# PrimeIntellect-ai/prime

Hardware: AMD Instinct MI355X
Metric: tokens_per_sec (higher is better)
Workload: dtype bf16; 1 GPU; model=intellect_10b, global_batch=8, seq_len=2048, parallelism=diloco1_h100_int8ring

## Files before the change

prime_amd/ops/_lib.py:

```python
from __future__ import annotations

import ctypes
from typing import Optional

import torch

from .build import LIB_PATH, build, needs_build

_LIB: Optional[ctypes.CDLL] = None
_TRIED = False

_SIGS = {
    "prime_rmsnorm_fwd": [ctypes.c_void_p] * 5 + [ctypes.c_int64] * 2 + [ctypes.c_double],
    "prime_rmsnorm_bwd": [ctypes.c_void_p] * 7 + [ctypes.c_int64] * 3 + [ctypes.c_double],
    "prime_add_rmsnorm_fwd": [ctypes.c_void_p] * 7 + [ctypes.c_int64] * 2 + [ctypes.c_double],
    "prime_add_rmsnorm_bwd": [ctypes.c_void_p] * 8 + [ctypes.c_int64] * 3 + [ctypes.c_double],
    "prime_rope": [ctypes.c_void_p] * 5 + [ctypes.c_int64] * 4 + [ctypes.c_int, ctypes.c_int64, ctypes.c_void_p],
    "prime_rope_strided": [ctypes.c_void_p] * 5 + [ctypes.c_int64] * 7,
    "prime_qkv_grad_pack": [ctypes.c_void_p] * 8 + [ctypes.c_int64] * 6,
    "prime_swiglu_bwd_t": [ctypes.c_void_p] * 5 + [ctypes.c_int64] * 2,
    "prime_swiglu_fwd": [ctypes.c_void_p] * 3 + [ctypes.c_int64] * 2,
    "prime_swiglu_bwd": [ctypes.c_void_p] * 4 + [ctypes.c_int64] * 2,
    "prime_adamw": [ctypes.c_void_p] * 7 + [ctypes.c_int64] + [ctypes.c_double] * 5 + [ctypes.c_int64],
    "prime_grad_sqnorm": [ctypes.c_void_p] * 3 + [ctypes.c_int64] * 2,
    "prime_grad_sqnorm_partials": [],
    "prime_pseudograd": [ctypes.c_void_p] * 4 + [ctypes.c_int64],
    "prime_quant_int8": [ctypes.c_void_p] * 4 + [ctypes.c_int64],
    "prime_dequant_int8": [ctypes.c_void_p] * 4 + [ctypes.c_int64] * 2,
    "prime_nesterov_outer": [ctypes.c_void_p] * 6 + [ctypes.c_int64] + [ctypes.c_double] * 2,
    "prime_cross_entropy": [ctypes.c_void_p] * 5 + [ctypes.c_int64] * 2 + [ctypes.c_double] + [ctypes.c_int64] * 2,
    "prime_flash_fwd": [ctypes.c_void_p] * 6 + [ctypes.c_int64] * 5 + [ctypes.c_double] + [ctypes.c_int64] * 7 + [ctypes.c_void_p],
    "prime_attn_delta": [ctypes.c_void_p] * 4 + [ctypes.c_int64] * 2,
    "prime_flash_bwd_dq": [ctypes.c_void_p] * 9 + [ctypes.c_int64] * 5 + [ctypes.c_double] + [ctypes.c_int64] * 10 + [ctypes.c_void_p],
    "prime_flash_bwd_dkv": [ctypes.c_void_p] * 13 + [ctypes.c_int64] * 6 + [ctypes.c_double] + [ctypes.c_int64] * 10 + [ctypes.c_void_p],
    "prime_mfma_probe": [ctypes.c_void_p] * 4,
    "prime_mfma_probe32": [ctypes.c_void_p] * 4,
    "prime_transpose_bshd": [ctypes.c_void_p] * 3 + [ctypes.c_int64] * 7,
    "prime_attn_decode": [ctypes.c_void_p] * 5 + [ctypes.c_int64] * 6 + [ctypes.c_double, ctypes.c_void_p],
    "prime_attn_decode_ragged": [ctypes.c_void_p] * 7 + [ctypes.c_int64] * 6 + [ctypes.c_double],
    "prime_decode_ragged_chunk": [],
    "prime_decode_qkv_append": [ctypes.c_void_p] * 8 + [ctypes.c_int64] * 6,
    "prime_gemm_nt": [ctypes.c_void_p] * 4 + [ctypes.c_int64] * 4,
    "prime_gemm_nt8": [ctypes.c_void_p] * 4 + [ctypes.c_int64] * 4,
    "prime_quant_fp8": [ctypes.c_void_p] * 6 + [ctypes.c_int64] * 2,
    "prime_rowwise_quant_fp8": [ctypes.c_void_p] * 4 + [ctypes.c_int64] * 3,
    "prime_transpose_fp8": [ctypes.c_void_p] * 3 + [ctypes.c_int64] * 7 + [ctypes.c_void_p] * 3 + [ctypes.c_int64],
}


def _load() -> ctypes.CDLL:
    import os

    override = os.environ.get("PRIME_AMD_LIB_PATH")
    path = override or str(LIB_PATH)
    if override is None and needs_build():
        build(verbose=True)
    lib = ctypes.CDLL(path)
    for name, argtypes in _SIGS.items():
        try:
            fn = getattr(lib, name)
        except AttributeError:
            continue
        fn.argtypes = argtypes
        fn.restype = ctypes.c_int
    return lib


def lib() -> ctypes.CDLL:
    global _LIB, _TRIED
    if _LIB is None:
        if _TRIED:
            raise RuntimeError("prime_amd HIP kernel library failed to load earlier")
        _TRIED = True
        try:
            _LIB = _load()
        except Exception as e:
            raise RuntimeError(
                "prime_amd requires its HIP kernel library on GPU machines; "
                f"build failed or .so missing at {LIB_PATH}: {e}"
            ) from e
    return _LIB


def have_lib() -> bool:
    try:
        lib()
        return True
# ... 19 lines not shown
```

prime_amd/ops/csrc/attention.hip:

```cpp
#include "common.h"
#include <stdlib.h>

typedef __attribute__((ext_vector_type(8))) short short8;
typedef __attribute__((ext_vector_type(4))) float f32x4;
typedef __attribute__((address_space(3))) char lds_char;
typedef __attribute__((address_space(3))) void lds_void;
typedef __attribute__((address_space(1))) const void g_void;

__device__ __forceinline__ short8 ld8(const bf16* p) {
  return *reinterpret_cast<const short8*>(p);
}

__device__ __forceinline__ f32x4 mfma16(short8 a, short8 b, f32x4 c) {
  return __builtin_amdgcn_mfma_f32_16x16x32_bf16(a, b, c, 0, 0, 0);
}

__device__ __forceinline__ float grp16_max(float x) {
#pragma unroll
  for (int off = 1; off < 16; off <<= 1) x = fmaxf(x, __shfl_xor(x, off, 64));
  return x;
}
__device__ __forceinline__ float grp16_sum(float x) {
#pragma unroll
  for (int off = 1; off < 16; off <<= 1) x += __shfl_xor(x, off, 64);
// ... 370 lines not shown
        psum += pv;
      }
    psum += __shfl_xor(psum, 32, 64);
    l_run = l_run * alpha + psum;

    short8 pa[2 * 2];
#pragma unroll
    for (int t = 0; t < 2; ++t) {
#pragma unroll
      for (int kst = 0; kst < 2; ++kst) {
        const int g0 = 4 * (2 * kst), g1 = 4 * (2 * kst + 1);
        unsigned x0 = cvt_pk_bf16(st[t][g0 + 0], st[t][g0 + 1]);
        unsigned x1 = cvt_pk_bf16(st[t][g0 + 2], st[t][g0 + 3]);
        unsigned y0 = cvt_pk_bf16(st[t][g1 + 0], st[t][g1 + 1]);
        unsigned y1 = cvt_pk_bf16(st[t][g1 + 2], st[t][g1 + 3]);
        permlane32_swap(x0, y0);
        permlane32_swap(x1, y1);
        short8 frag;
        reinterpret_cast<unsigned*>(&frag)[0] = x0;
        reinterpret_cast<unsigned*>(&frag)[1] = x1;
        reinterpret_cast<unsigned*>(&frag)[2] = y0;
        reinterpret_cast<unsigned*>(&frag)[3] = y1;
        pa[t * 2 + kst] = frag;
      }
    }
    if (FLAGS & 1) __builtin_amdgcn_s_setprio(1);
#pragma unroll
    for (int dt = 0; dt < DT32; ++dt)
#pragma unroll
      for (int ks = 0; ks < 4; ++ks)
        o_acc[dt] = mfma32(pa[ks],
                           ld8_swz<64>(vt_lds[idx], dt * 32 + lo, ks * 32 + hi * 16),
                           o_acc[dt]);
    if (FLAGS & 1) __builtin_amdgcn_s_setprio(0);
  }
  if (hi == 0) bcast[lo] = (l_run > 0.f) ? 1.f / l_run : 0.f;
  wave_lds_fence();
#pragma unroll
  for (int r = 0; r < 16; ++r) {
    const int qr = (r & 3) + 8 * (r >> 2) + 4 * hi;
    const float inv = bcast[qr];
    bf16* orow = O + (((int64_t)(b * S + q0w + qr)) * H + h) * D;
#pragma unroll
    for (int dt = 0; dt < DT32; ++dt)
      orow[dt * 32 + lo] = f2bf(o_acc[dt][r] * inv);
  }
  if (hi == 0)
    lse[((int64_t)(b * S + q0w + lo)) * H + h] = m_run + __logf(fmaxf(l_run, 1e-30f));
}

__global__ void attn_delta_kernel(const bf16* __restrict__ dO,
                                  const bf16* __restrict__ O,
                                  float* __restrict__ delta, int64_t rows,
                                  int D) {
  const int64_t row0 = (int64_t)blockIdx.x * (blockDim.x >> 6) + (threadIdx.x >> 6);
  const int lane = threadIdx.x & 63;
  for (int64_t r = row0; r < rows; r += (int64_t)gridDim.x * (blockDim.x >> 6)) {
    float acc = 0.f;
    for (int i = lane * 2; i < D; i += 128) {
      acc += bf2f(dO[r * D + i]) * bf2f(O[r * D + i]);
      acc += bf2f(dO[r * D + i + 1]) * bf2f(O[r * D + i + 1]);
    }
    acc = wave_reduce_sum(acc);
    if (lane == 0) delta[r] = acc;
  }
}

template <int D, int FLAGS, bool DOC = false>
__global__ __launch_bounds__(512, 2) void flash_bwd_dq_v5_kernel(
    const bf16* __restrict__ Q, const bf16* __restrict__ K,
    const bf16* __restrict__ V, const bf16* __restrict__ Kt,
    const bf16* __restrict__ dO, const float* __restrict__ lse,
    const float* __restrict__ delta, bf16* __restrict__ dQ, int B, int H,
    int Hkv, int S, float scale, int causal,
    int64_t sqb, int64_t sqs, int64_t sqh,
    int64_t skb, int64_t sks, int64_t skh,
    int64_t svb, int64_t svs, int64_t svh,
    const int* __restrict__ doc) {
  constexpr int DSL = D / 16;
  constexpr int DT32 = D / 32;
  const int n_qt = S / 256;
  const int nwg = gridDim.x;
  int vb = blockIdx.x;
  if ((nwg & 7) == 0) vb = (blockIdx.x & 7) * (nwg >> 3) + (blockIdx.x >> 3);
  const int bh = vb / n_qt;
  const int qt = n_qt - 1 - (vb - bh * n_qt);
  const int b = bh / H, h = bh - b * H;
  const int hkv = h / (H / Hkv);
  const int wid = threadIdx.x >> 6;
  const int lane = threadIdx.x & 63;
  const int lo = lane & 31, hi = lane >> 5;
  const int q0w = qt * 256 + wid * 32;

  const bf16* Qb = Q + b * sqb + h * sqh;
  const bf16* Kb = K + b * skb + hkv * skh;
  const bf16* Vb = V + b * svb + hkv * svh;
  const bf16* Ktb = Kt + ((int64_t)(b * Hkv + hkv) * D) * S;
  const bf16* dOb = dO + ((int64_t)b * S * H + h) * D;
  const float* lse_b = lse + (int64_t)b * S * H + h;
  const float* dl_b = delta + (int64_t)b * S * H + h;

  __shared__ bf16 k_lds[2][64 * D];
  __shared__ bf16 v_lds[2][64 * D];
  __shared__ bf16 kt_lds[2][D * 64];

  short8 qf[DSL], dof[DSL];
#pragma unroll
  for (int ds = 0; ds < DSL; ++ds) {
    const bf16* src = Qb + (int64_t)(q0w + lo) * sqs + ds * 16 + hi * 8;
    short8 raw = ld8(src);
    short8 sc;
#pragma unroll
    for (int j = 0; j < 8; ++j) {
      bf16 v = reinterpret_cast<const bf16*>(&raw)[j];
      reinterpret_cast<bf16*>(&sc)[j] = f2bf(bf2f(v) * scale);
    }
    qf[ds] = sc;
// ... 308 lines not shown
        const int g0 = 4 * (2 * kst), g1 = 4 * (2 * kst + 1);
        unsigned x0 = cvt_pk_bf16(st[g0 + 0], st[g0 + 1]);
        unsigned x1 = cvt_pk_bf16(st[g0 + 2], st[g0 + 3]);
        unsigned y0 = cvt_pk_bf16(st[g1 + 0], st[g1 + 1]);
        unsigned y1 = cvt_pk_bf16(st[g1 + 2], st[g1 + 3]);
        permlane32_swap(x0, y0);
        permlane32_swap(x1, y1);
        short8 f;
        reinterpret_cast<unsigned*>(&f)[0] = x0;
        reinterpret_cast<unsigned*>(&f)[1] = x1;
        reinterpret_cast<unsigned*>(&f)[2] = y0;
        reinterpret_cast<unsigned*>(&f)[3] = y1;
        pa[kst] = f;
        x0 = cvt_pk_bf16(dpt[g0 + 0], dpt[g0 + 1]);
        x1 = cvt_pk_bf16(dpt[g0 + 2], dpt[g0 + 3]);
        y0 = cvt_pk_bf16(dpt[g1 + 0], dpt[g1 + 1]);
        y1 = cvt_pk_bf16(dpt[g1 + 2], dpt[g1 + 3]);
        permlane32_swap(x0, y0);
        permlane32_swap(x1, y1);
        reinterpret_cast<unsigned*>(&f)[0] = x0;
        reinterpret_cast<unsigned*>(&f)[1] = x1;
        reinterpret_cast<unsigned*>(&f)[2] = y0;
        reinterpret_cast<unsigned*>(&f)[3] = y1;
        da[kst] = f;
      }
      if (FLAGS & 1) __builtin_amdgcn_s_setprio(1);
#pragma unroll
      for (int dt = 0; dt < DT32; ++dt)
#pragma unroll
        for (int kst = 0; kst < 2; ++kst) {
          const int colb = qs * 64 + kst * 32 + hi * 16;
          dv_acc[dt] = mfma32(pa[kst],
                              ld8_swz<64>(dot_lds[cur], dt * 32 + lo, colb),
                              dv_acc[dt]);
          dk_acc[dt] = mfma32(da[kst],
                              ld8_swz<64>(qt_lds[cur], dt * 32 + lo, colb),
                              dk_acc[dt]);
        }
      if (FLAGS & 1) __builtin_amdgcn_s_setprio(0);
    }
  }
#pragma unroll
  for (int r = 0; r < 16; ++r) {
    const int kg = k0w + (r & 3) + 8 * (r >> 2) + 4 * hi;
    const int64_t base = ((((int64_t)split * B + b) * Hkv + hkv) * S + kg) * D;
#pragma unroll
    for (int dt = 0; dt < DT32; ++dt) {
      wsK[base + dt * 32 + lo] = dk_acc[dt][r];
      wsV[base + dt * 32 + lo] = dv_acc[dt][r];
    }
  }
}

template <int D, int NW = 4, int DBUF = 1, bool DOC = false>
__global__ __launch_bounds__(512) void flash_bwd_dkv_kernel(
    const bf16* __restrict__ Q, const bf16* __restrict__ Qt,
    const bf16* __restrict__ K, const bf16* __restrict__ V,
    const bf16* __restrict__ dO, const bf16* __restrict__ dOt,
    const float* __restrict__ lse, const float* __restrict__ delta,
    float* __restrict__ wsK, float* __restrict__ wsV, int B, int H, int Hkv,
    int S, float scale, int causal, int splits,
    int64_t sqb, int64_t sqs, int64_t sqh,
    int64_t skb, int64_t sks, int64_t skh,
    int64_t svb, int64_t svs, int64_t svh,
    const int* __restrict__ doc_end) {
  constexpr int DS = D / 32;
  constexpr int DT = D / 16;
  const int n_kt = S / (NW * 16);
  const int per_split = (B * Hkv) * n_kt;
  const int split = blockIdx.x / per_split;
  const int rem = blockIdx.x - split * per_split;
  const int bh = rem / n_kt;
  const int kt = rem - bh * n_kt;
  const int b = bh / Hkv, hkv = bh - b * Hkv;
  const int group = H / Hkv;
  const int wid = threadIdx.x >> 6;
  const int lane = threadIdx.x & 63;
  const int lg = lane >> 4, li = lane & 15;
  const int k0 = kt * (NW * 16) + wid * 16;

  const bf16* Kb = K + b * skb + hkv * skh;
  const bf16* Vb = V + b * svb + hkv * svh;

  __shared__ bf16 q_lds[DBUF][64 * D];
  __shared__ bf16 do_lds[DBUF][64 * D];
  __shared__ bf16 qt_lds[DBUF][D * 64];
  __shared__ bf16 dot_lds[DBUF][D * 64];
  __shared__ bf16 pt_lds_all[NW][16 * 64];
  __shared__ bf16 dst_lds_all[NW][16 * 64];
  bf16* pt_lds = pt_lds_all[wid];
  bf16* dst_lds = dst_lds_all[wid];

  short8 kf[DS], vf[DS];
#pragma unroll
  for (int ds = 0; ds < DS; ++ds) {
    kf[ds] = ld8(Kb + (int64_t)(k0 + li) * sks + ds * 32 + lg * 8);
    vf[ds] = ld8(Vb + (int64_t)(k0 + li) * svs + ds * 32 + lg * 8);
  }
  f32x4 dk_acc[DT], dv_acc[DT];
#pragma unroll
  for (int dt = 0; dt < DT; ++dt) {
    dk_acc[dt] = f32x4{0.f, 0.f, 0.f, 0.f};
    dv_acc[dt] = f32x4{0.f, 0.f, 0.f, 0.f};
  }

  const int q_start = (causal ? (kt * (NW * 16)) / 64 * 64 : 0) + split * 64;
  int q_end = S, my_q_end = S, key_end[4];
  if (DOC) {
    const int* de_b = doc_end + (int64_t)b * S;
    q_end = (doc_clamp(de_b[kt * (NW * 16) + NW * 16 - 1], S) + 63) & ~63;
    my_q_end = doc_clamp(de_b[k0 + 15], S);
#pragma unroll
    for (int r = 0; r < 4; ++r) key_end[r] = de_b[k0 + lg * 4 + r];
  }
  const int tiles_per_g =
      (q_end > q_start) ? (q_end - q_start + 64 * splits - 1) / (64 * splits) : 0;
  const int n_iter = group * tiles_per_g;
  const auto stage_it = [&](int it, int buf) {
    const int g_ = it / tiles_per_g;
    const int q0g_ = q_start + (it - g_ * tiles_per_g) * 64 * splits;
    const int h_ = hkv * group + g_;
    const bf16* Qb_ = Q + b * sqb + h_ * sqh;
    const bf16* dOb_ = dO + ((int64_t)b * S * H + h_) * D;
    const bf16* Qtb_ = Qt + ((int64_t)(b * H + h_) * D) * S;
    const bf16* dOtb_ = dOt + ((int64_t)(b * H + h_) * D) * S;
    stage_tile<64, D, NW * 64>(Qb_ + (int64_t)q0g_ * sqs, sqs, q_lds[buf], threadIdx.x);
    stage_tile<64, D, NW * 64>(dOb_ + (int64_t)q0g_ * H * D, (int64_t)H * D, do_lds[buf], threadIdx.x);
    stage_tile<D, 64, NW * 64>(Qtb_ + q0g_, S, qt_lds[buf], threadIdx.x);
    stage_tile<D, 64, NW * 64>(dOtb_ + q0g_, S, dot_lds[buf], threadIdx.x);
  };
  if (DBUF == 2 && n_iter > 0) stage_it(0, 0);
  for (int it = 0; it < n_iter; ++it) {
    const int g = it / tiles_per_g;
    const int q0g = q_start + (it - g * tiles_per_g) * 64 * splits;
    const int h = hkv * group + g;
    const float* lse_b = lse + (int64_t)b * S * H + h;
    const float* dl_b = delta + (int64_t)b * S * H + h;
    const int cur = (DBUF == 2) ? (it & 1) : 0;
    {
      __syncthreads();
      if (DBUF == 2) {
        if (it + 1 < n_iter) stage_it(it + 1, cur ^ 1);
      } else {
        stage_it(it, 0);
        __syncthreads();
      }
      if (causal && q0g + 64 <= k0) continue;
      if (DOC && q0g >= my_q_end) continue;
#pragma unroll
      for (int sub = 0; sub < 4; ++sub) {
        f32x4 st_acc{0.f, 0.f, 0.f, 0.f}, dpt_acc{0.f, 0.f, 0.f, 0.f};
#pragma unroll
        for (int ds = 0; ds < DS; ++ds) {
          const short8 qb = ld8_swz<D>(q_lds[cur], sub * 16 + li, ds * 64 + lg * 16);
          const short8 dob = ld8_swz<D>(do_lds[cur], sub * 16 + li, ds * 64 + lg * 16);
          st_acc = mfma16(kf[ds], qb, st_acc);
          dpt_acc = mfma16(vf[ds], dob, dpt_acc);
        }
        const int qg = q0g + sub * 16 + li;
        const float lse_q = lse_b[(int64_t)qg * H];
        const float dl_q = dl_b[(int64_t)qg * H];
#pragma unroll
        for (int r = 0; r < 4; ++r) {
          const int kg = k0 + lg * 4 + r;
          float p = __expf(st_acc[r] * scale - lse_q);
          if (causal && kg > qg) p = 0.f;
          if (DOC && qg >= key_end[r]) p = 0.f;
          st16_swz<64>(pt_lds, lg * 4 + r, sub * 16 + li, f2bf(p));
          st16_swz<64>(dst_lds, lg * 4 + r, sub * 16 + li,
                       f2bf(p * (dpt_acc[r] - dl_q) * scale));
        }
      }
      wave_lds_fence();
#pragma unroll
      for (int dt = 0; dt < DT; ++dt)
#pragma unroll
        for (int ks = 0; ks < 2; ++ks) {
          const short8 pa = ld8_swz<64>(pt_lds, li, ks * 64 + lg * 16);
          const short8 da = ld8_swz<64>(dst_lds, li, ks * 64 + lg * 16);
          dv_acc[dt] = mfma16(pa, ld8_swz<64>(dot_lds[cur], dt * 16 + li, ks * 64 + lg * 16), dv_acc[dt]);
          dk_acc[dt] = mfma16(da, ld8_swz<64>(qt_lds[cur], dt * 16 + li, ks * 64 + lg * 16), dk_acc[dt]);
        }
    }
  }
#pragma unroll
  for (int r = 0; r < 4; ++r) {
    const int kg = k0 + lg * 4 + r;
    const int64_t base = ((((int64_t)split * B + b) * Hkv + hkv) * S + kg) * D;
#pragma unroll
    for (int dt = 0; dt < DT; ++dt) {
      wsK[base + dt * 16 + li] = dk_acc[dt][r];
      wsV[base + dt * 16 + li] = dv_acc[dt][r];
    }
  }
}

__global__ void dkv_reduce_kernel(const float* __restrict__ wsK,
                                  const float* __restrict__ wsV,
                                  bf16* __restrict__ dK, bf16* __restrict__ dV,
                                  int B, int Hkv, int S, int D, int splits) {
  const int64_t n = (int64_t)B * Hkv * S * D;
  for (int64_t i = (int64_t)blockIdx.x * blockDim.x + threadIdx.x; i < n;
       i += (int64_t)gridDim.x * blockDim.x) {
    float k = 0.f, v = 0.f;
    for (int sp = 0; sp < splits; ++sp) {
      k += wsK[(int64_t)sp * n + i];
      v += wsV[(int64_t)sp * n + i];
    }
    const int d = (int)(i % D);
    int64_t r = i / D;
    const int sq = (int)(r % S);
    r /= S;
    const int hk = (int)(r % Hkv);
    const int bb = (int)(r / Hkv);
    const int64_t o = (((int64_t)(bb * S + sq)) * Hkv + hk) * D + d;
    dK[o] = f2bf(k);
    dV[o] = f2bf(v);
  }
}

#define DISPATCH_D(KER, ...)                                            \
  do {                                                                  \
    if (D == 128)                                                       \
      hipLaunchKernelGGL(KER<128>, dim3(grid), dim3(256), 0, stream,    \
                         __VA_ARGS__);                                  \
    else                                                                \
      hipLaunchKernelGGL(KER<64>, dim3(grid), dim3(256), 0, stream,     \
                         __VA_ARGS__);                                  \
  } while (0)

PRIME_API int prime_flash_fwd(hipStream_t stream, const void* Q, const void* K,
                              const void* Vt, void* O, void* lse, int64_t B,
                              int64_t H, int64_t Hkv, int64_t S, int64_t D,
                              double scale, int64_t causal,
                              int64_t sqb, int64_t sqs, int64_t sqh,
                              int64_t skb, int64_t sks, int64_t skh,
                              const void* doc_start) {
  if (S % 64 != 0 || (D != 64 && D != 128)) return hipErrorInvalidValue;
  static const char* v5env = getenv("PRIME_ATTN_V5");
  static const char* flagenv = getenv("PRIME_ATTN_FLAGS");
  if (doc_start) {
    if (!causal) return hipErrorInvalidValue;
    const bool v5 = (S % 256 == 0) && !(v5env && v5env[0] == '0');
#define LAUNCH_FWD_DOC(KER, QT, NT)                                          \
    hipLaunchKernelGGL(KER, dim3((int)(B * H * (S / QT))), dim3(NT), 0,      \
                       stream, (const bf16*)Q, (const bf16*)K,               \
// ... 20 lines not shown
                           (float)scale, (int)causal, sqb, sqs, sqh, skb,
                           sks, skh, (const int*)nullptr);
        break;
      default:
        hipLaunchKernelGGL((flash_fwd_v5_kernel<64, 2>), dim3(grid),
                           dim3(512), 0, stream, (const bf16*)Q,
                           (const bf16*)K, (const bf16*)Vt, (bf16*)O,
                           (float*)lse, (int)B, (int)H, (int)Hkv, (int)S,
                           (float)scale, (int)causal, sqb, sqs, sqh, skb,
                           sks, skh, (const int*)nullptr);
        break;
    }
    return (int)hipGetLastError();
  }
  if (use_v5) {
    const int grid = (int)(B * H * (S / 256));
#define LAUNCH_V5(F)                                                         \
    hipLaunchKernelGGL((flash_fwd_v5_kernel<128, F>), dim3(grid), dim3(512), \
                       0, stream, (const bf16*)Q, (const bf16*)K,            \
                       (const bf16*)Vt, (bf16*)O, (float*)lse, (int)B,       \
                       (int)H, (int)Hkv, (int)S, (float)scale, (int)causal,  \
                       sqb, sqs, sqh, skb, sks, skh, (const int*)nullptr)
    switch (flags & 7) {
      case 0: LAUNCH_V5(0); break;
      case 1: LAUNCH_V5(1); break;
      case 2: LAUNCH_V5(2); break;
      case 3: LAUNCH_V5(3); break;
      case 6: LAUNCH_V5(6); break;
      case 7: LAUNCH_V5(7); break;
      default: LAUNCH_V5(2); break;
    }
    return (int)hipGetLastError();
  }
#define LAUNCH_FWD(DD, NW)                                                  \
  hipLaunchKernelGGL((flash_fwd_kernel<DD, NW>), dim3(grid),                \
                     dim3(NW * 64), 0, stream, (const bf16*)Q,              \
                     (const bf16*)K, (const bf16*)Vt, (bf16*)O, (float*)lse,\
                     (int)B, (int)H, (int)Hkv, (int)S, (float)scale,        \
                     (int)causal, sqb, sqs, sqh, skb, sks, skh,              \
                     (const int*)nullptr)
  {
    const int grid = (int)(B * H * (S / 64));
    if (D == 128) LAUNCH_FWD(128, 4); else LAUNCH_FWD(64, 4);
  }
  return (int)hipGetLastError();
}

PRIME_API int prime_attn_delta(hipStream_t stream, const void* dO,
                               const void* O, void* delta, int64_t rows,
                               int64_t D) {
  int grid = prime_grid(rows * 64, 256);
  hipLaunchKernelGGL(attn_delta_kernel, dim3(grid), dim3(256), 0, stream,
                     (const bf16*)dO, (const bf16*)O, (float*)delta, rows,
                     (int)D);
  return (int)hipGetLastError();
}

PRIME_API int prime_flash_bwd_dq(hipStream_t stream, const void* Q,
                                 const void* K, const void* V, const void* Kt,
                                 const void* dO, const void* lse,
                                 const void* delta, void* dQ, int64_t B,
                                 int64_t H, int64_t Hkv, int64_t S, int64_t D,
                                 double scale, int64_t causal,
                                 int64_t sqb, int64_t sqs, int64_t sqh,
                                 int64_t skb, int64_t sks, int64_t skh,
                                 int64_t svb, int64_t svs, int64_t svh,
                                 const void* doc_start) {
  if (S % 64 != 0 || (D != 64 && D != 128)) return hipErrorInvalidValue;
  static const char* v5env = getenv("PRIME_ATTN_V5");
  static const char* flagenv = getenv("PRIME_ATTN_FLAGS");
  const int flags = flagenv ? atoi(flagenv) : 2;
  if (doc_start) {
    if (!causal) return hipErrorInvalidValue;
    const bool v5 = (S % 256 == 0) && !(v5env && v5env[0] == '0');
#define LAUNCH_DQ_DOC(KER, QT, NT)                                           \
    hipLaunchKernelGGL(KER, dim3((int)(B * H * (S / QT))), dim3(NT), 0,      \
                       stream, (const bf16*)Q, (const bf16*)K,               \
                       (const bf16*)V, (const bf16*)Kt, (const bf16*)dO,     \
                       (const float*)lse, (const float*)delta, (bf16*)dQ,    \
                       (int)B, (int)H, (int)Hkv, (int)S, (float)scale, 1,    \
                       sqb, sqs, sqh, skb, sks, skh, svb, svs, svh,          \
                       (const int*)doc_start)
    if (v5 && D == 128) LAUNCH_DQ_DOC((flash_bwd_dq_v5_kernel<128, 0, true>), 256, 512);
    else if (v5) LAUNCH_DQ_DOC((flash_bwd_dq_v5_kernel<64, 0, true>), 256, 512);
    else if (D == 128) LAUNCH_DQ_DOC((flash_bwd_dq_kernel<128, true>), 64, 256);
    else LAUNCH_DQ_DOC((flash_bwd_dq_kernel<64, true>), 64, 256);
    return (int)hipGetLastError();
  }
  if ((D == 64) && (S % 256 == 0) && !(v5env && v5env[0] == '0')) {
    const int grid = (int)(B * H * (S / 256));
    hipLaunchKernelGGL((flash_bwd_dq_v5_kernel<64, 0>), dim3(grid),
                       dim3(512), 0, stream, (const bf16*)Q, (const bf16*)K,
                       (const bf16*)V, (const bf16*)Kt, (const bf16*)dO,
                       (const float*)lse, (const float*)delta, (bf16*)dQ,
                       (int)B, (int)H, (int)Hkv, (int)S, (float)scale,
                       (int)causal, sqb, sqs, sqh, skb, sks, skh,
                       svb, svs, svh, (const int*)nullptr);
    return (int)hipGetLastError();
  }
  if ((D == 128) && (S % 256 == 0) && !(v5env && v5env[0] == '0')) {
    const int grid = (int)(B * H * (S / 256));
#define LAUNCH_DQ5(F)                                                       \
    hipLaunchKernelGGL((flash_bwd_dq_v5_kernel<128, F>), dim3(grid),        \
                       dim3(512), 0, stream, (const bf16*)Q,                \
                       (const bf16*)K, (const bf16*)V, (const bf16*)Kt,     \
                       (const bf16*)dO, (const float*)lse,                  \
                       (const float*)delta, (bf16*)dQ, (int)B, (int)H,      \
                       (int)Hkv, (int)S, (float)scale, (int)causal,         \
                       sqb, sqs, sqh, skb, sks, skh, svb, svs, svh,         \
                       (const int*)nullptr)
    if (flags & 1) LAUNCH_DQ5(1); else LAUNCH_DQ5(0);
    return (int)hipGetLastError();
  }
  const int grid = (int)(B * H * (S / 64));
  DISPATCH_D(flash_bwd_dq_kernel, (const bf16*)Q, (const bf16*)K,
             (const bf16*)V, (const bf16*)Kt, (const bf16*)dO,
             (const float*)lse, (const float*)delta, (bf16*)dQ, (int)B, (int)H,
             (int)Hkv, (int)S, (float)scale, (int)causal, sqb, sqs, sqh, skb,
             sks, skh, svb, svs, svh, (const int*)nullptr);
  return (int)hipGetLastError();
}

PRIME_API int prime_flash_bwd_dkv(hipStream_t stream, const void* Q,
                                  const void* Qt, const void* K, const void* V,
                                  const void* dO, const void* dOt,
                                  const void* lse, const void* delta, void* dK,
                                  void* dV, void* wsK, void* wsV,
                                  int64_t splits, int64_t B, int64_t H,
                                  int64_t Hkv, int64_t S, int64_t D,
                                  double scale, int64_t causal,
                                  int64_t sqb, int64_t sqs, int64_t sqh,
                                  int64_t skb, int64_t sks, int64_t skh,
                                  int64_t svb, int64_t svs, int64_t svh,
                                  const void* doc_end) {
  if (S % 64 != 0 || (D != 64 && D != 128)) return hipErrorInvalidValue;
  if (doc_end && !causal) return hipErrorInvalidValue;
  static const char* v5denv = getenv("PRIME_ATTN_DKV5");
  static const char* fenv = getenv("PRIME_ATTN_FLAGS");
  const int flags = fenv ? atoi(fenv) : 2;
  if (!doc_end && (D == 128) && (S % 256 == 0) && (v5denv && v5denv[0] == '1')) {
    const int sp = (int)(splits > 4 ? 4 : splits);
    const int grid = (int)(B * Hkv * (S / 256) * sp);
#define LAUNCH_DKV5(F)                                                       \
    hipLaunchKernelGGL((flash_bwd_dkv_v5_kernel<128, F>), dim3(grid),        \
                       dim3(512), 0, stream, (const bf16*)Q,                 \
                       (const bf16*)Qt, (const bf16*)K, (const bf16*)V,      \
                       (const bf16*)dO, (const bf16*)dOt,                    \
                       (const float*)lse, (const float*)delta, (float*)wsK,  \
                       (float*)wsV, (int)B, (int)H, (int)Hkv, (int)S,        \
                       (float)scale, (int)causal, sp, sqb, sqs, sqh,         \
                       skb, sks, skh, svb, svs, svh)
    if (flags & 1) LAUNCH_DKV5(1); else LAUNCH_DKV5(0);
    int err5 = hipGetLastError();
    if (err5) return err5;
    int rgrid5 = prime_grid(B * Hkv * S * D, 256);
    hipLaunchKernelGGL(dkv_reduce_kernel, dim3(rgrid5), dim3(256), 0, stream,
                       (const float*)wsK, (const float*)wsV, (bf16*)dK,
                       (bf16*)dV, (int)B, (int)Hkv, (int)S, (int)D, sp);
    return (int)hipGetLastError();
  }
  static const char* nw8env = getenv("PRIME_ATTN_DKV8");
  const bool nw8 = (S % 128 == 0) && !(nw8env && nw8env[0] == '0');
#define LAUNCH_DKV(DD, NWV, DB) LAUNCH_DKV_(DD, NWV, DB, false, nullptr)
#define LAUNCH_DKV_DOC(DD, NWV, DB) LAUNCH_DKV_(DD, NWV, DB, true, doc_end)
#define LAUNCH_DKV_(DD, NWV, DB, DOCV, DOCP)                                 \
    hipLaunchKernelGGL((flash_bwd_dkv_kernel<DD, NWV, DB, DOCV>),            \
                       dim3((int)(B * Hkv * (S / (NWV * 16)) * splits)),     \
                       dim3(NWV * 64), 0, stream, (const bf16*)Q,            \
                       (const bf16*)Qt, (const bf16*)K, (const bf16*)V,      \
                       (const bf16*)dO, (const bf16*)dOt,                    \
                       (const float*)lse, (const float*)delta, (float*)wsK,  \
                       (float*)wsV, (int)B, (int)H, (int)Hkv, (int)S,        \
                       (float)scale, (int)causal, (int)splits, sqb, sqs,     \
                       sqh, skb, sks, skh, svb, svs, svh, (const int*)DOCP)
  static const char* dbenv = getenv("PRIME_ATTN_DKV_DBUF");
  const bool dbuf = !(dbenv && dbenv[0] == '0');
  if (doc_end) {
    if (nw8 && dbuf) {
      if (D == 128) LAUNCH_DKV_DOC(128, 8, 2); else LAUNCH_DKV_DOC(64, 8, 2);
    } else if (nw8) {
      if (D == 128) LAUNCH_DKV_DOC(128, 8, 1); else LAUNCH_DKV_DOC(64, 8, 1);
    } else {
      if (D == 128) LAUNCH_DKV_DOC(128, 4, 1); else LAUNCH_DKV_DOC(64, 4, 1);
    }
  } else if (nw8 && dbuf) {
    if (D == 128) LAUNCH_DKV(128, 8, 2); else LAUNCH_DKV(64, 8, 2);
  } else if (nw8) {
    if (D == 128) LAUNCH_DKV(128, 8, 1); else LAUNCH_DKV(64, 8, 1);
  } else {
    if (D == 128) LAUNCH_DKV(128, 4, 1); else LAUNCH_DKV(64, 4, 1);
  }
  int err = hipGetLastError();
  if (err) return err;
  int rgrid = prime_grid(B * Hkv * S * D, 256);
  hipLaunchKernelGGL(dkv_reduce_kernel, dim3(rgrid), dim3(256), 0, stream,
                     (const float*)wsK, (const float*)wsV, (bf16*)dK,
                     (bf16*)dV, (int)B, (int)Hkv, (int)S, (int)D, (int)splits);
  return (int)hipGetLastError();
}
```

prime_amd/ops/functional.py:

```python
from __future__ import annotations

import torch

from . import reference as ref
from ._lib import check, lib, ptr, stream_of

_DW_ROWS = 1024


def _is_hip(t: torch.Tensor) -> bool:
    return t.is_cuda


class _RMSNorm(torch.autograd.Function):
    @staticmethod
    def forward(ctx, x: torch.Tensor, w: torch.Tensor, eps: float):
        if not _is_hip(x):
            ctx.save_for_backward(x, w)
            ctx.eps = eps
            return ref.rmsnorm(x, w, eps)
        x = x.contiguous()
        shp = x.shape
        D = shp[-1]
        if D % 8 != 0:
# ... 264 lines not shown
    if not causal:
        raise ValueError("flash_attention: doc_start requires causal=True")
    if not isinstance(doc_start, torch.Tensor) or doc_start.dtype != torch.int32:
        raise TypeError(
            "flash_attention: doc_start must be an int32 tensor "
            f"(got {getattr(doc_start, 'dtype', type(doc_start))})")
    if tuple(doc_start.shape) != (B, S):
        raise ValueError(
            f"flash_attention: doc_start must have shape [B, S] = [{B}, {S}] "
            f"(got {list(doc_start.shape)})")
    if doc_start.device != q.device:
        raise ValueError(
            f"flash_attention: doc_start is on {doc_start.device}, q on {q.device}")


class _FlashAttention(torch.autograd.Function):

    @staticmethod
    def forward(ctx, q, k, v, causal: bool, scale: float, doc_start=None):
        B, S, H, D = q.shape
        _check_flash_shape(S, D)
        Hkv = k.shape[2]
        if not (_bshd_ok(q) and _bshd_ok(k) and _bshd_ok(v)):
            q, k, v = q.contiguous(), k.contiguous(), v.contiguous()
        if doc_start is not None:
            doc_start = doc_start.contiguous()
        vt = transpose_bshd(v)
        o = torch.empty(B, S, H, D, device=q.device, dtype=q.dtype)
        lse = torch.empty(B, S, H, device=q.device, dtype=torch.float32)
        check(
            lib().prime_flash_fwd(
                stream_of(q), ptr(q), ptr(k), ptr(vt), ptr(o), ptr(lse),
                B, H, Hkv, S, D, scale, int(causal),
                q.stride(0), q.stride(1), q.stride(2),
                k.stride(0), k.stride(1), k.stride(2), ptr(doc_start),
            ),
            "flash_fwd",
        )
        ctx.save_for_backward(q, k, v, o, lse)
        ctx.meta = (causal, scale)
        ctx.doc_start = doc_start
        return o

    @staticmethod
    def backward(ctx, do):
        q, k, v, o, lse = ctx.saved_tensors
        causal, scale = ctx.meta
        doc_start = ctx.doc_start
        doc_end = _doc_ends_cached(doc_start) if doc_start is not None else None
        B, S, H, D = q.shape
        Hkv = k.shape[2]
        do = do.contiguous()
        delta = torch.empty(B * S * H, device=q.device, dtype=torch.float32)
        check(
            lib().prime_attn_delta(stream_of(q), ptr(do), ptr(o), ptr(delta), B * S * H, D),
            "attn_delta",
        )
        kt = transpose_bshd(k)
        dq = torch.empty(B, S, H, D, device=q.device, dtype=q.dtype)
        check(
            lib().prime_flash_bwd_dq(
                stream_of(q), ptr(q), ptr(k), ptr(v), ptr(kt), ptr(do),
                ptr(lse), ptr(delta), ptr(dq), B, H, Hkv, S, D, scale,
                int(causal),
                q.stride(0), q.stride(1), q.stride(2),
                k.stride(0), k.stride(1), k.stride(2),
                v.stride(0), v.stride(1), v.stride(2), ptr(doc_start),
            ),
            "flash_bwd_dq",
        )
        qt = transpose_bshd(q)
        dot = transpose_bshd(do)
        dk = torch.empty(B, S, Hkv, D, device=q.device, dtype=q.dtype)
        dv = torch.empty(B, S, Hkv, D, device=q.device, dtype=q.dtype)
        import os

        env = os.environ.get("PRIME_AMD_DKV_SPLITS")
        if env:
            splits = max(1, min(int(env), S // 64))
        else:
            splits = max(1, min(8, S // 1024, S // 64))
        ws = torch.empty(2, splits, B, Hkv, S, D, device=q.device,
                         dtype=torch.float32)
        check(
            lib().prime_flash_bwd_dkv(
                stream_of(q), ptr(q), ptr(qt), ptr(k), ptr(v), ptr(do),
                ptr(dot), ptr(lse), ptr(delta), ptr(dk), ptr(dv),
                ptr(ws[0]), ptr(ws[1]), splits,
                B, H, Hkv, S, D, scale, int(causal),
                q.stride(0), q.stride(1), q.stride(2),
                k.stride(0), k.stride(1), k.stride(2),
                v.stride(0), v.stride(1), v.stride(2), ptr(doc_end),
            ),
            "flash_bwd_dkv",
        )
        return dq, dk, dv, None, None, None


def flash_attention(q, k, v, causal: bool = True, doc_start=None) -> torch.Tensor:
    if doc_start is not None:
        _check_doc_start(doc_start, q, causal)
    if not _is_hip(q):
        return ref.attention(q, k, v, causal, doc_start=doc_start)
    if doc_start is None:
        return _FlashAttention.apply(q, k, v, causal, q.shape[-1] ** -0.5)
    return _FlashAttention.apply(q, k, v, causal, q.shape[-1] ** -0.5, doc_start)


class _CrossEntropy(torch.autograd.Function):
    @staticmethod
    def forward(ctx, logits, targets, ignore_index: int, need_grad: bool):
        R, V = logits.shape
        logits = logits.contiguous()
        t32 = targets.to(torch.int32).contiguous()
        loss = torch.empty(R, device=logits.device, dtype=torch.float32)
        dlogits = torch.empty_like(logits) if need_grad else logits
        check(
            lib().prime_cross_entropy(
                stream_of(logits), ptr(logits), ptr(t32), ptr(loss), ptr(dlogits),
                R, V, 1.0, ignore_index, 1 if need_grad else 0,
            ),
            "cross_entropy",
        )
        n_valid = (targets != ignore_index).sum().clamp(min=1)
        if need_grad:
            ctx.save_for_backward(dlogits, n_valid)
        else:
            ctx.save_for_backward(torch.empty(0, device=logits.device,
                                              dtype=logits.dtype), n_valid)
        return loss.sum() / n_valid.float()

    @staticmethod
    def backward(ctx, grad_out):
        dlogits, n_valid = ctx.saved_tensors
        g = dlogits * (grad_out.float() / n_valid.float()).to(dlogits.dtype)
        return g, None, None, None


def cross_entropy(logits, targets, ignore_index: int = -100) -> torch.Tensor:
    if not _is_hip(logits):
        return ref.cross_entropy(logits, targets, ignore_index)
# ... 638 lines not shown
```

Before: 15930 tokens/s.

## Add direct-write paired-tile dK/dV backward with transposed lse/delta row constants

The attention delta kernel now also writes lse and delta into a [2,B,H,S] transposed buffer, so the dK/dV kernel can read per-query constants contiguously (vector loads) instead of with stride H. When the block count already fills the GPU, a new direct mode has each block loop over the splits itself, pairing causal key tiles (kt, n_kt-1-kt) to balance work, and accumulating in a single workspace slice before writing bf16 dK/dV, which skips the separate reduce kernel and the large multi-split fp32 workspace. An optional key-per-lane variant that keeps P/dS in registers is added but disabled by default. The trade-off is fewer, longer blocks with serialized split passes and an extra fp32 read/write per split.

```diff
diff --git a/prime_amd/ops/_lib.py b/prime_amd/ops/_lib.py
--- a/prime_amd/ops/_lib.py
+++ b/prime_amd/ops/_lib.py
@@ -32,7 +32,9 @@
     "prime_flash_fwd": [ctypes.c_void_p] * 6 + [ctypes.c_int64] * 5 + [ctypes.c_double] + [ctypes.c_int64] * 7 + [ctypes.c_void_p],
     "prime_attn_delta": [ctypes.c_void_p] * 4 + [ctypes.c_int64] * 2,
     "prime_flash_bwd_dq": [ctypes.c_void_p] * 9 + [ctypes.c_int64] * 5 + [ctypes.c_double] + [ctypes.c_int64] * 10 + [ctypes.c_void_p],
-    "prime_flash_bwd_dkv": [ctypes.c_void_p] * 13 + [ctypes.c_int64] * 6 + [ctypes.c_double] + [ctypes.c_int64] * 10 + [ctypes.c_void_p],
+    "prime_attn_delta_t": [ctypes.c_void_p] * 6 + [ctypes.c_int64] * 4,
+    "prime_flash_bwd_dkv": [ctypes.c_void_p] * 14 + [ctypes.c_int64] * 6 + [ctypes.c_double] + [ctypes.c_int64] * 10 + [ctypes.c_void_p],
+    "prime_flash_bwd_dkv_direct": [ctypes.c_int64] * 6,
     "prime_mfma_probe": [ctypes.c_void_p] * 4,
     "prime_mfma_probe32": [ctypes.c_void_p] * 4,
     "prime_transpose_bshd": [ctypes.c_void_p] * 3 + [ctypes.c_int64] * 7,
diff --git a/prime_amd/ops/csrc/attention.hip b/prime_amd/ops/csrc/attention.hip
--- a/prime_amd/ops/csrc/attention.hip
+++ b/prime_amd/ops/csrc/attention.hip
@@ -446,7 +446,8 @@
 __global__ void attn_delta_kernel(const bf16* __restrict__ dO,
                                   const bf16* __restrict__ O,
                                   float* __restrict__ delta, int64_t rows,
-                                  int D) {
+                                  int D, const float* __restrict__ lse,
+                                  float* __restrict__ rowc_t, int S, int H) {
   const int64_t row0 = (int64_t)blockIdx.x * (blockDim.x >> 6) + (threadIdx.x >> 6);
   const int lane = threadIdx.x & 63;
   for (int64_t r = row0; r < rows; r += (int64_t)gridDim.x * (blockDim.x >> 6)) {
@@ -456,7 +457,18 @@
       acc += bf2f(dO[r * D + i + 1]) * bf2f(O[r * D + i + 1]);
     }
     acc = wave_reduce_sum(acc);
-    if (lane == 0) delta[r] = acc;
+    if (lane == 0) {
+      delta[r] = acc;
+      if (rowc_t) {
+        const int64_t bs = r / H;
+        const int h = (int)(r - bs * H);
+        const int64_t bb = bs / S;
+        const int s = (int)(bs - bb * S);
+        const int64_t t = (bb * H + h) * S + s;
+        rowc_t[t] = lse[r];
+        rowc_t[rows + t] = acc;
+      }
+    }
   }
 }
 
@@ -871,14 +883,40 @@
   }
 }
 
+__device__ __forceinline__ short8 ld4x2_swz(const bf16* lds_tile, int row,
+                                            int colb) {
+  typedef __attribute__((ext_vector_type(4))) short short4v;
+  const char* base = reinterpret_cast<const char*>(lds_tile) + row * 128;
+  const int sw = (row & 7) << 4;
+  const short4v lo = *reinterpret_cast<const short4v*>(base + (colb ^ sw));
+  const short4v hi = *reinterpret_cast<const short4v*>(base + ((colb + 32) ^ sw));
+  return __builtin_shufflevector(lo, hi, 0, 1, 2, 3, 4, 5, 6, 7);
+}
+
+__device__ __forceinline__ short bf_bits(bf16 x) {
+  return (short)__bfloat16_as_ushort(x);
+}
+
+#ifndef PRIME_DKV_KEYLANE
+#define PRIME_DKV_KEYLANE 0
+#endif
+#ifndef PRIME_DKV_ROWC_PREFETCH
+#define PRIME_DKV_ROWC_PREFETCH 1
+#endif
+#if !PRIME_DKV_KEYLANE
+#undef PRIME_DKV_ROWC_PREFETCH
+#define PRIME_DKV_ROWC_PREFETCH 0
+#endif
+
 template <int D, int NW = 4, int DBUF = 1, bool DOC = false>
 __global__ __launch_bounds__(512) void flash_bwd_dkv_kernel(
     const bf16* __restrict__ Q, const bf16* __restrict__ Qt,
     const bf16* __restrict__ K, const bf16* __restrict__ V,
     const bf16* __restrict__ dO, const bf16* __restrict__ dOt,
-    const float* __restrict__ lse, const float* __restrict__ delta,
-    float* __restrict__ wsK, float* __restrict__ wsV, int B, int H, int Hkv,
-    int S, float scale, int causal, int splits,
+    const float* __restrict__ rowc,
+    float* __restrict__ wsK, float* __restrict__ wsV,
+    bf16* __restrict__ dK, bf16* __restrict__ dV, int B, int H, int Hkv,
+    int S, float scale, int causal, int splits, int direct,
     int64_t sqb, int64_t sqs, int64_t sqh,
     int64_t skb, int64_t sks, int64_t skh,
     int64_t svb, int64_t svs, int64_t svh,
@@ -886,29 +924,44 @@
   constexpr int DS = D / 32;
   constexpr int DT = D / 16;
   const int n_kt = S / (NW * 16);
-  const int per_split = (B * Hkv) * n_kt;
-  const int split = blockIdx.x / per_split;
-  const int rem = blockIdx.x - split * per_split;
-  const int bh = rem / n_kt;
-  const int kt = rem - bh * n_kt;
+  const bool paired = direct && causal;
+  const int per_bh = paired ? (n_kt + 1) / 2 : n_kt;
+  const int per_split = (B * Hkv) * per_bh;
+  const int blk_split = blockIdx.x / per_split;
+  const int rem = blockIdx.x - blk_split * per_split;
+  const int bh = rem / per_bh;
+  const int kt0 = rem - bh * per_bh;
+  const int n_pass = (paired && kt0 != n_kt - 1 - kt0) ? 2 : 1;
   const int b = bh / Hkv, hkv = bh - b * Hkv;
   const int group = H / Hkv;
   const int wid = threadIdx.x >> 6;
   const int lane = threadIdx.x & 63;
   const int lg = lane >> 4, li = lane & 15;
-  const int k0 = kt * (NW * 16) + wid * 16;
 
   const bf16* Kb = K + b * skb + hkv * skh;
   const bf16* Vb = V + b * svb + hkv * svh;
+  const float* lse_t = rowc + (int64_t)b * H * S;
+  const float* dl_t = lse_t + (int64_t)B * H * S;
 
   __shared__ bf16 q_lds[DBUF][64 * D];
   __shared__ bf16 do_lds[DBUF][64 * D];
   __shared__ bf16 qt_lds[DBUF][D * 64];
   __shared__ bf16 dot_lds[DBUF][D * 64];
+#if !PRIME_DKV_KEYLANE
   __shared__ bf16 pt_lds_all[NW][16 * 64];
   __shared__ bf16 dst_lds_all[NW][16 * 64];
   bf16* pt_lds = pt_lds_all[wid];
   bf16* dst_lds = dst_lds_all[wid];
+#endif
+
+  const int n_vs = direct ? splits : 1;
+  for (int pv = 0; pv < n_pass * n_vs; ++pv) {
+  const int pass = pv / n_vs;
+  const int vs = pv - pass * n_vs;
+  const int split = direct ? vs : blk_split;
+  const int kt = pass ? n_kt - 1 - kt0 : kt0;
+  const int k0 = kt * (NW * 16) + wid * 16;
+  if (pv) __syncthreads();
 
   short8 kf[DS], vf[DS];
 #pragma unroll
@@ -924,14 +977,20 @@
   }
 
   const int q_start = (causal ? (kt * (NW * 16)) / 64 * 64 : 0) + split * 64;
-  int q_end = S, my_q_end = S, key_end[4];
+  int q_end = S, my_q_end = S, key_end = S;
   if (DOC) {
     const int* de_b = doc_end + (int64_t)b * S;
     q_end = (doc_clamp(de_b[kt * (NW * 16) + NW * 16 - 1], S) + 63) & ~63;
     my_q_end = doc_clamp(de_b[k0 + 15], S);
-#pragma unroll
-    for (int r = 0; r < 4; ++r) key_end[r] = de_b[k0 + lg * 4 + r];
-  }
+    key_end = de_b[k0 + li];
+  }
+#if !PRIME_DKV_KEYLANE
+  int key_end4[4] = {S, S, S, S};
+  if (DOC) {
+#pragma unroll
+    for (int r = 0; r < 4; ++r) key_end4[r] = doc_end[(int64_t)b * S + k0 + lg * 4 + r];
+  }
+#endif
   const int tiles_per_g =
       (q_end > q_start) ? (q_end - q_start + 64 * splits - 1) / (64 * splits) : 0;
   const int n_iter = group * tiles_per_g;
@@ -948,14 +1007,26 @@
     stage_tile<D, 64, NW * 64>(Qtb_ + q0g_, S, qt_lds[buf], threadIdx.x);
     stage_tile<D, 64, NW * 64>(dOtb_ + q0g_, S, dot_lds[buf], threadIdx.x);
   };
+  const auto rowc_off = [&](int it, int sub) {
+    const int g_ = it / tiles_per_g;
+    const int q0g_ = q_start + (it - g_ * tiles_per_g) * 64 * splits;
+    return (int64_t)(hkv * group + g_) * S + q0g_ + sub * 16 + lg * 4;
+  };
+  f32x4 lse_r[4], dl_r[4];
+  if (PRIME_DKV_ROWC_PREFETCH && n_iter > 0) {
+#pragma unroll
+    for (int sub = 0; sub < 4; ++sub) {
+      const int64_t o = rowc_off(0, sub);
+      lse_r[sub] = *reinterpret_cast<const f32x4*>(lse_t + o);
+      dl_r[sub] = *reinterpret_cast<const f32x4*>(dl_t + o);
+    }
+  }
   if (DBUF == 2 && n_iter > 0) stage_it(0, 0);
   for (int it = 0; it < n_iter; ++it) {
     const int g = it / tiles_per_g;
     const int q0g = q_start + (it - g * tiles_per_g) * 64 * splits;
-    const int h = hkv * group + g;
-    const float* lse_b = lse + (int64_t)b * S * H + h;
-    const float* dl_b = delta + (int64_t)b * S * H + h;
     const int cur = (DBUF == 2) ? (it & 1) : 0;
+    const int itn = (it + 1 < n_iter) ? it + 1 : it;
     {
       __syncthreads();
       if (DBUF == 2) {
@@ -964,8 +1035,19 @@
         stage_it(it, 0);
         __syncthreads();
       }
-      if (causal && q0g + 64 <= k0) continue;
-      if (DOC && q0g >= my_q_end) continue;
+      const bool skip = (causal && q0g + 64 <= k0) || (DOC && q0g >= my_q_end);
+      if (skip) {
+        if (PRIME_DKV_ROWC_PREFETCH) {
+#pragma unroll
+          for (int sub = 0; sub < 4; ++sub) {
+            const int64_t o = rowc_off(itn, sub);
+            lse_r[sub] = *reinterpret_cast<const f32x4*>(lse_t + o);
+            dl_r[sub] = *reinterpret_cast<const f32x4*>(dl_t + o);
+          }
+        }
+        continue;
+      }
+#if !PRIME_DKV_KEYLANE
 #pragma unroll
       for (int sub = 0; sub < 4; ++sub) {
         f32x4 st_acc{0.f, 0.f, 0.f, 0.f}, dpt_acc{0.f, 0.f, 0.f, 0.f};
@@ -977,14 +1059,14 @@
           dpt_acc = mfma16(vf[ds], dob, dpt_acc);
         }
         const int qg = q0g + sub * 16 + li;
-        const float lse_q = lse_b[(int64_t)qg * H];
-        const float dl_q = dl_b[(int64_t)qg * H];
+        const int64_t o = (int64_t)(hkv * group + g) * S + qg;
+        const float lse_q = lse_t[o];
+        const float dl_q = dl_t[o];
 #pragma unroll
         for (int r = 0; r < 4; ++r) {
-          const int kg = k0 + lg * 4 + r;
           float p = __expf(st_acc[r] * scale - lse_q);
-          if (causal && kg > qg) p = 0.f;
-          if (DOC && qg >= key_end[r]) p = 0.f;
+          if (causal && k0 + lg * 4 + r > qg) p = 0.f;
+          if (DOC && qg >= key_end4[r]) p = 0.f;
           st16_swz<64>(pt_lds, lg * 4 + r, sub * 16 + li, f2bf(p));
           st16_swz<64>(dst_lds, lg * 4 + r, sub * 16 + li,
                        f2bf(p * (dpt_acc[r] - dl_q) * scale));
@@ -1000,17 +1082,116 @@
           dv_acc[dt] = mfma16(pa, ld8_swz<64>(dot_lds[cur], dt * 16 + li, ks * 64 + lg * 16), dv_acc[dt]);
           dk_acc[dt] = mfma16(da, ld8_swz<64>(qt_lds[cur], dt * 16 + li, ks * 64 + lg * 16), dk_acc[dt]);
         }
-    }
-  }
+#else
+#pragma unroll
+      for (int c = 0; c < 2; ++c) {
+        short8 pb, dsb;
+#pragma unroll
+        for (int s2 = 0; s2 < 2; ++s2) {
+          const int sub = c * 2 + s2;
+          f32x4 s_acc{0.f, 0.f, 0.f, 0.f}, dp_acc{0.f, 0.f, 0.f, 0.f};
+#pragma unroll
+          for (int ds = 0; ds < DS; ++ds) {
+            const short8 qb = ld8_swz<D>(q_lds[cur], sub * 16 + li, ds * 64 + lg * 16);
+            const short8 dob = ld8_swz<D>(do_lds[cur], sub * 16 + li, ds * 64 + lg * 16);
+            s_acc = mfma16(qb, kf[ds], s_acc);
+            dp_acc = mfma16(dob, vf[ds], dp_acc);
+          }
+          f32x4 lse_q, dl_q;
+          if (PRIME_DKV_ROWC_PREFETCH) {
+            lse_q = lse_r[sub];
+            dl_q = dl_r[sub];
+            const int64_t o = rowc_off(itn, sub);
+            lse_r[sub] = *reinterpret_cast<const f32x4*>(lse_t + o);
+            dl_r[sub] = *reinterpret_cast<const f32x4*>(dl_t + o);
+          } else {
+            const int64_t o = rowc_off(it, sub);
+            lse_q = *reinterpret_cast<const f32x4*>(lse_t + o);
+            dl_q = *reinterpret_cast<const f32x4*>(dl_t + o);
+          }
+#pragma unroll
+          for (int r = 0; r < 4; ++r) {
+            const int qg = q0g + sub * 16 + lg * 4 + r;
+            float p = __expf(s_acc[r] * scale - lse_q[r]);
+            if (causal && k0 + li > qg) p = 0.f;
+            if (DOC && qg >= key_end) p = 0.f;
+            pb[s2 * 4 + r] = bf_bits(f2bf(p));
+            dsb[s2 * 4 + r] = bf_bits(f2bf(p * (dp_acc[r] - dl_q[r]) * scale));
+          }
+        }
+#pragma unroll
+        for (int dt = 0; dt < DT; ++dt) {
+          const short8 dota = ld4x2_swz(dot_lds[cur], dt * 16 + li, c * 64 + lg * 8);
+          const short8 qta = ld4x2_swz(qt_lds[cur], dt * 16 + li, c * 64 + lg * 8);
+          dv_acc[dt] = mfma16(dota, pb, dv_acc[dt]);
+          dk_acc[dt] = mfma16(qta, dsb, dk_acc[dt]);
+        }
+      }
+#endif
+    }
+  }
+#if !PRIME_DKV_KEYLANE
 #pragma unroll
   for (int r = 0; r < 4; ++r) {
-    const int kg = k0 + lg * 4 + r;
-    const int64_t base = ((((int64_t)split * B + b) * Hkv + hkv) * S + kg) * D;
+    const int kr = k0 + lg * 4 + r;
+    const int64_t ob = (((int64_t)b * S + kr) * Hkv + hkv) * D + li;
+    const int64_t wb = ((((int64_t)blk_split * B + b) * Hkv + hkv) * S + kr) * D + li;
 #pragma unroll
     for (int dt = 0; dt < DT; ++dt) {
-      wsK[base + dt * 16 + li] = dk_acc[dt][r];
-      wsV[base + dt * 16 + li] = dv_acc[dt][r];
-    }
+      if (direct) {
+        float sk = 0.f + dk_acc[dt][r], sv = 0.f + dv_acc[dt][r];
+        if (vs > 0) {
+          sk = wsK[wb + dt * 16] + dk_acc[dt][r];
+          sv = wsV[wb + dt * 16] + dv_acc[dt][r];
+        }
+        if (vs + 1 < n_vs) {
+          wsK[wb + dt * 16] = sk;
+          wsV[wb + dt * 16] = sv;
+        } else {
+          dK[ob + dt * 16] = f2bf(sk);
+          dV[ob + dt * 16] = f2bf(sv);
+        }
+      } else {
+        wsK[wb + dt * 16] = dk_acc[dt][r];
+        wsV[wb + dt * 16] = dv_acc[dt][r];
+      }
+    }
+  }
+#else
+  const int kg = k0 + li;
+  const int64_t wbase = ((((int64_t)blk_split * B + b) * Hkv + hkv) * S + kg) * D + lg * 4;
+  if (direct) {
+    const int64_t base = (((int64_t)b * S + kg) * Hkv + hkv) * D + lg * 4;
+    const f32x4 zero{0.f, 0.f, 0.f, 0.f};
+#pragma unroll
+    for (int dt = 0; dt < DT; ++dt) {
+      f32x4 sk = zero + dk_acc[dt], sv = zero + dv_acc[dt];
+      if (vs > 0) {
+        sk = *reinterpret_cast<f32x4*>(wsK + wbase + dt * 16) + dk_acc[dt];
+        sv = *reinterpret_cast<f32x4*>(wsV + wbase + dt * 16) + dv_acc[dt];
+      }
+      if (vs + 1 < n_vs) {
+        *reinterpret_cast<f32x4*>(wsK + wbase + dt * 16) = sk;
+        *reinterpret_cast<f32x4*>(wsV + wbase + dt * 16) = sv;
+      } else {
+        bf16x4 ok, ov;
+#pragma unroll
+        for (int r = 0; r < 4; ++r) {
+          ok.v[r] = f2bf(sk[r]);
+          ov.v[r] = f2bf(sv[r]);
+        }
+        *reinterpret_cast<bf16x4*>(dK + base + dt * 16) = ok;
+        *reinterpret_cast<bf16x4*>(dV + base + dt * 16) = ov;
+      }
+    }
+  } else {
+#pragma unroll
+    for (int dt = 0; dt < DT; ++dt) {
+      *reinterpret_cast<f32x4*>(wsK + wbase + dt * 16) = dk_acc[dt];
+      *reinterpret_cast<f32x4*>(wsV + wbase + dt * 16) = dv_acc[dt];
+    }
+  }
+#endif
   }
 }
 
@@ -1137,7 +1318,20 @@
   int grid = prime_grid(rows * 64, 256);
   hipLaunchKernelGGL(attn_delta_kernel, dim3(grid), dim3(256), 0, stream,
                      (const bf16*)dO, (const bf16*)O, (float*)delta, rows,
-                     (int)D);
+                     (int)D, (const float*)nullptr, (float*)nullptr, 1, 1);
+  return (int)hipGetLastError();
+}
+
+PRIME_API int prime_attn_delta_t(hipStream_t stream, const void* dO,
+                                 const void* O, const void* lse, void* delta,
+                                 void* rowc_t, int64_t B, int64_t S, int64_t H,
+                                 int64_t D) {
+  if (!lse || !rowc_t) return hipErrorInvalidValue;
+  const int64_t rows = B * S * H;
+  int grid = prime_grid(rows * 64, 256);
+  hipLaunchKernelGGL(attn_delta_kernel, dim3(grid), dim3(256), 0, stream,
+                     (const bf16*)dO, (const bf16*)O, (float*)delta, rows,
+                     (int)D, (const float*)lse, (float*)rowc_t, (int)S, (int)H);
   return (int)hipGetLastError();
 }
 
@@ -1206,10 +1400,42 @@
   return (int)hipGetLastError();
 }
 
+static bool dkv_v5_selected(bool doc, int64_t D, int64_t S) {
+  static const char* v5denv = getenv("PRIME_ATTN_DKV5");
+  return !doc && (D == 128) && (S % 256 == 0) && (v5denv && v5denv[0] == '1');
+}
+
+static bool dkv_nw8(int64_t S) {
+  static const char* nw8env = getenv("PRIME_ATTN_DKV8");
+  return (S % 128 == 0) && !(nw8env && nw8env[0] == '0');
+}
+
+PRIME_API int prime_flash_bwd_dkv_direct(int64_t B, int64_t Hkv, int64_t S,
+                                         int64_t D, int64_t causal,
+                                         int64_t has_doc) {
+  if (dkv_v5_selected(has_doc != 0, D, S)) return 0;
+  const char* env = getenv("PRIME_ATTN_DKV_DIRECT");
+  if (env && env[0] == '1') return 1;
+  if (env && env[0] == '0') return 0;
+  static int n_cu = 0;
+  if (n_cu == 0) {
+    int dev = 0, n = 0;
+    if (hipGetDevice(&dev) != hipSuccess ||
+        hipDeviceGetAttribute(&n, hipDeviceAttributeMultiprocessorCount, dev) != hipSuccess ||
+        n <= 0)
+      n = 256;
+    n_cu = n;
+  }
+  const int64_t n_kt = S / (dkv_nw8(S) ? 128 : 64);
+  const int64_t blocks = B * Hkv * (causal ? (n_kt + 1) / 2 : n_kt);
+  return blocks >= n_cu ? 1 : 0;
+}
+
 PRIME_API int prime_flash_bwd_dkv(hipStream_t stream, const void* Q,
                                   const void* Qt, const void* K, const void* V,
                                   const void* dO, const void* dOt,
-                                  const void* lse, const void* delta, void* dK,
+                                  const void* lse, const void* delta,
+                                  const void* rowc, void* dK,
                                   void* dV, void* wsK, void* wsV,
                                   int64_t splits, int64_t B, int64_t H,
                                   int64_t Hkv, int64_t S, int64_t D,
@@ -1220,10 +1446,13 @@
                                   const void* doc_end) {
   if (S % 64 != 0 || (D != 64 && D != 128)) return hipErrorInvalidValue;
   if (doc_end && !causal) return hipErrorInvalidValue;
-  static const char* v5denv = getenv("PRIME_ATTN_DKV5");
   static const char* fenv = getenv("PRIME_ATTN_FLAGS");
   const int flags = fenv ? atoi(fenv) : 2;
-  if (!doc_end && (D == 128) && (S % 256 == 0) && (v5denv && v5denv[0] == '1')) {
+  const bool direct =
+      prime_flash_bwd_dkv_direct(B, Hkv, S, D, causal, doc_end != nullptr) != 0;
+  if (splits < 1) return hipErrorInvalidValue;
+  if ((!direct || splits > 1) && (!wsK || !wsV)) return hipErrorInvalidValue;
+  if (dkv_v5_selected(doc_end != nullptr, D, S)) {
     const int sp = (int)(splits > 4 ? 4 : splits);
     const int grid = (int)(B * Hkv * (S / 256) * sp);
 #define LAUNCH_DKV5(F)                                                       \
@@ -1244,20 +1473,23 @@
                        (bf16*)dV, (int)B, (int)Hkv, (int)S, (int)D, sp);
     return (int)hipGetLastError();
   }
-  static const char* nw8env = getenv("PRIME_ATTN_DKV8");
-  const bool nw8 = (S % 128 == 0) && !(nw8env && nw8env[0] == '0');
+  if (!rowc) return hipErrorInvalidValue;
+  const bool nw8 = dkv_nw8(S);
+  const int64_t n_kt = S / (nw8 ? 128 : 64);
+  const int64_t per_bh = (direct && causal) ? (n_kt + 1) / 2 : n_kt;
 #define LAUNCH_DKV(DD, NWV, DB) LAUNCH_DKV_(DD, NWV, DB, false, nullptr)
 #define LAUNCH_DKV_DOC(DD, NWV, DB) LAUNCH_DKV_(DD, NWV, DB, true, doc_end)
 #define LAUNCH_DKV_(DD, NWV, DB, DOCV, DOCP)                                 \
     hipLaunchKernelGGL((flash_bwd_dkv_kernel<DD, NWV, DB, DOCV>),            \
-                       dim3((int)(B * Hkv * (S / (NWV * 16)) * splits)),     \
+                       dim3((int)(B * Hkv * per_bh * (direct ? 1 : splits))), \
                        dim3(NWV * 64), 0, stream, (const bf16*)Q,            \
                        (const bf16*)Qt, (const bf16*)K, (const bf16*)V,      \
                        (const bf16*)dO, (const bf16*)dOt,                    \
-                       (const float*)lse, (const float*)delta, (float*)wsK,  \
-                       (float*)wsV, (int)B, (int)H, (int)Hkv, (int)S,        \
-                       (float)scale, (int)causal, (int)splits, sqb, sqs,     \
-                       sqh, skb, sks, skh, svb, svs, svh, (const int*)DOCP)
+                       (const float*)rowc, (float*)wsK, (float*)wsV,         \
+                       (bf16*)dK, (bf16*)dV, (int)B, (int)H, (int)Hkv,       \
+                       (int)S, (float)scale, (int)causal, (int)splits,       \
+                       (int)direct, sqb, sqs, sqh, skb, sks, skh, svb, svs,  \
+                       svh, (const int*)DOCP)
   static const char* dbenv = getenv("PRIME_ATTN_DKV_DBUF");
   const bool dbuf = !(dbenv && dbenv[0] == '0');
   if (doc_end) {
@@ -1276,7 +1508,7 @@
     if (D == 128) LAUNCH_DKV(128, 4, 1); else LAUNCH_DKV(64, 4, 1);
   }
   int err = hipGetLastError();
-  if (err) return err;
+  if (err || direct) return err;
   int rgrid = prime_grid(B * Hkv * S * D, 256);
   hipLaunchKernelGGL(dkv_reduce_kernel, dim3(rgrid), dim3(256), 0, stream,
                      (const float*)wsK, (const float*)wsV, (bf16*)dK,
diff --git a/prime_amd/ops/functional.py b/prime_amd/ops/functional.py
--- a/prime_amd/ops/functional.py
+++ b/prime_amd/ops/functional.py
@@ -340,8 +340,10 @@
         Hkv = k.shape[2]
         do = do.contiguous()
         delta = torch.empty(B * S * H, device=q.device, dtype=torch.float32)
-        check(
-            lib().prime_attn_delta(stream_of(q), ptr(do), ptr(o), ptr(delta), B * S * H, D),
+        rowc = torch.empty(2, B, H, S, device=q.device, dtype=torch.float32)
+        check(
+            lib().prime_attn_delta_t(stream_of(q), ptr(do), ptr(o), ptr(lse), ptr(delta),
+                                     ptr(rowc), B, S, H, D),
             "attn_delta",
         )
         kt = transpose_bshd(k)
@@ -363,18 +365,21 @@
         dv = torch.empty(B, S, Hkv, D, device=q.device, dtype=q.dtype)
         import os
 
+        direct = bool(lib().prime_flash_bwd_dkv_direct(
+            B, Hkv, S, D, int(causal), int(doc_end is not None)))
         env = os.environ.get("PRIME_AMD_DKV_SPLITS")
         if env:
             splits = max(1, min(int(env), S // 64))
         else:
             splits = max(1, min(8, S // 1024, S // 64))
-        ws = torch.empty(2, splits, B, Hkv, S, D, device=q.device,
-                         dtype=torch.float32)
+        ws_slices = (0 if splits == 1 else 1) if direct else splits
+        ws = torch.empty(2, ws_slices, B, Hkv, S, D, device=q.device,
+                         dtype=torch.float32) if ws_slices else None
         check(
             lib().prime_flash_bwd_dkv(
                 stream_of(q), ptr(q), ptr(qt), ptr(k), ptr(v), ptr(do),
-                ptr(dot), ptr(lse), ptr(delta), ptr(dk), ptr(dv),
-                ptr(ws[0]), ptr(ws[1]), splits,
+                ptr(dot), ptr(lse), ptr(delta), ptr(rowc), ptr(dk), ptr(dv),
+                ptr(None if ws is None else ws[0]), ptr(None if ws is None else ws[1]), splits,
                 B, H, Hkv, S, D, scale, int(causal),
                 q.stride(0), q.stride(1), q.stride(2),
                 k.stride(0), k.stride(1), k.stride(2),
```

After: 16520 tokens/s, median of 6. 1.04x the previous value.
